# davidfang00/opticalflowdiffusion

Measured on AMD Instinct MI355X. Metric: UNet denoise steps/sec @ 2x436x1024 flow, bs=16, higher is better.
Workload: dtype bf16

## Files before the change

opticalflowdiffusion_amd/csrc/la_fused.hip:

```cpp
#include <cstdlib>
#include "blocks.h"

namespace ofd {

int la_fused_blocks(int n, int B);

typedef __attribute__((ext_vector_type(8))) __bf16 bf16x8;
typedef __attribute__((ext_vector_type(16))) float f32x16;

__device__ __forceinline__ uint32_t la_pack2(float a, float b) { return f2bf2(a, b); }
__device__ __forceinline__ int acc_row(int r, int half) { return (r & 3) + 8 * (r >> 2) + 4 * half; }

__device__ __forceinline__ bf16x8 acc_frag(const f32x16& a, int s2) {
    bf16x8 f;
#pragma unroll
    for (int j = 0; j < 8; ++j) f[j] = (__bf16)a[8 * s2 + j];
    return f;
}

typedef __attribute__((ext_vector_type(4))) unsigned int u32x4;
template <int C>
struct XRaw {
    u32x4 v[C / 16];
};
// ... 327 lines not shown
    __syncthreads();
    const bool use_ws = nparts <= LA_MAX_PARTS;
    float l = 0.0f;
    for (int c0 = grp; c0 < nparts; c0 += 32) {
        float tm[4], tl[4];
#pragma unroll
        for (int k = 0; k < 4; ++k) {
            const size_t o = (size_t)min(c0 + 8 * k, nparts - 1) * 1088;
            tm[k] = base[o + dd];
            tl[k] = base[o + 32 + dd];
        }
#pragma unroll
        for (int k = 0; k < 4; ++k)
            if (c0 + 8 * k < nparts) {
                const float w = __expf(tm[k] - M[dd]);
                if (use_ws) w_s[c0 + 8 * k][dd] = w;
                l += tl[k] * w;
            }
    }
    __syncthreads();
    red[grp][dd] = l;
    __syncthreads();
    if (tid < 32) {
        float t = red[0][tid];
#pragma unroll
        for (int g = 1; g < 8; ++g) t += red[g][tid];
        Linv[tid] = 1.0f / t;
    }
    __syncthreads();
    const int i = blockIdx.y * 256 + tid;
    const int j = i & 7, lane = (i >> 3) & 63, s2 = i >> 9;
    const int d = 16 * s2 + 8 * (j >> 2) + 4 * (lane >> 5) + (j & 3), e = lane & 31;
    float a = 0.0f;
    for (int c0 = 0; c0 < nparts; c0 += 8) {
        float v[8];
#pragma unroll
        for (int k = 0; k < 8; ++k) v[k] = base[(size_t)min(c0 + k, nparts - 1) * 1088 + 64 + d * 32 + e];
        if (use_ws) {
#pragma unroll
            for (int k = 0; k < 8; ++k)
                if (c0 + k < nparts) a += v[k] * w_s[c0 + k][d];
        } else {
            float mc[8];
#pragma unroll
            for (int k = 0; k < 8; ++k) mc[k] = base[(size_t)min(c0 + k, nparts - 1) * 1088 + d];
#pragma unroll
            for (int k = 0; k < 8; ++k)
                if (c0 + k < nparts) a += v[k] * __expf(mc[k] - M[d]);
        }
    }
    ctxfrag[(size_t)bh * 1024 + i] = f2bf(a * Linv[d] * inv_n);
}

template <int C, bool TRAIN>
__global__ void __launch_bounds__(256, C == 64 ? 4 : 2) la_out_fused_kernel(const bf16_t* __restrict__ x, const bf16_t* __restrict__ wq,
                                                           const bf16_t* __restrict__ woutp, const bf16_t* __restrict__ ctxfrag,
                                                           const float* __restrict__ bias, const float* __restrict__ g2,
                                                           bf16_t* __restrict__ y, int n, float eps_pre, float eps_post, float scale,
                                                           const float* __restrict__ g, bf16_t* __restrict__ o2_out) {
    extern __shared__ __attribute__((aligned(16))) unsigned char smem[];
    constexpr int KS = C / 16, RT = C / 32;
    constexpr int WQ_B = (C / 8) * 128 * 16, WO_B = 16 * C * 16, CF_B = 4 * 2 * 64 * 16;
    unsigned char* s_wq = smem;
    unsigned char* s_wo = smem + WQ_B;
    unsigned char* s_cf = s_wo + WO_B;
    float* s_bias = (float*)(s_cf + CF_B);
    float* s_g2 = s_bias + C;
    float* s_g = s_g2 + C;
    const int tid = threadIdx.x, lane = tid & 63, wave = tid >> 6, l31 = lane & 31, half = lane >> 5;
    const int b = blockIdx.y;
    if constexpr (TRAIN)
        for (int i = tid; i < C; i += 256) s_g[i] = g[i];
    for (int i = tid; i < WQ_B / 16; i += 256) ((uint4*)s_wq)[i] = ((const uint4*)wq)[i];
    for (int i = tid; i < WO_B / 16; i += 256) ((uint4*)s_wo)[i] = ((const uint4*)woutp)[i];
    for (int i = tid; i < CF_B / 16; i += 256) ((uint4*)s_cf)[i] = ((const uint4*)(ctxfrag + (size_t)b * 4096))[i];
    for (int i = tid; i < C; i += 256) { s_bias[i] = bias[i]; s_g2[i] = g2[i]; }
    __syncthreads();
    const int wave_id = blockIdx.x * 4 + wave, nw = gridDim.x * 4, ntiles = (n + 31) / 32;

    const bf16_t* xb = x + (size_t)b * n * C;
    XRaw<C> raw_next;
    load_raw_x<C>(xb + (size_t)min(wave_id * 32 + l31, n - 1) * C, raw_next, half);
    for (int tile = wave_id; tile < ntiles; tile += nw) {
        asm volatile("" ::: "memory");
        const int pix = tile * 32 + l31;
        const int pid = min(pix, n - 1);
        const bf16_t* xrow = xb + (size_t)pid * C;
        const XRaw<C> raw = raw_next;
        load_raw_x<C>(xb + (size_t)min((tile + nw) * 32 + l31, n - 1) * C, raw_next, half);
        bf16x8 xs[KS];
        if constexpr (TRAIN) norm_x_gain<C>(raw, eps_pre, s_g, half, xs);
        else norm_x<C>(raw, eps_pre, xs);
        f32x16 acc_o[RT];
#pragma unroll
        for (int rt = 0; rt < RT; ++rt)
#pragma unroll
            for (int r = 0; r < 16; ++r) acc_o[rt][r] = 0.0f;
#pragma unroll
        for (int hd = 0; hd < 4; ++hd) {
            f32x16 qa;
#pragma unroll
            for (int r = 0; r < 16; ++r) qa[r] = 0.0f;
#pragma unroll
            for (int s = 0; s < KS; ++s) {
                const bf16x8 wf = *(const bf16x8*)(s_wq + ((size_t)(2 * s + half) * 128 + hd * 32 + l31) * 16);
                qa = __builtin_amdgcn_mfma_f32_32x32x16_bf16(wf, xs[s], qa, 0, 0, 0);
            }
            if constexpr (TRAIN) {
#pragma unroll
                for (int r = 0; r < 16; ++r) qa[r] = bf2f(f2bf(qa[r]));
            }
            float mx = qa[0];
#pragma unroll
            for (int r = 1; r < 16; ++r) mx = fmaxf(mx, qa[r]);
            mx = fmaxf(mx, __shfl_xor(mx, 32, 64));
            float sum = 0.0f;
#pragma unroll
            for (int r = 0; r < 16; ++r) { qa[r] = __builtin_amdgcn_exp2f(__builtin_fmaf(qa[r], LOG2E, -mx * LOG2E)); sum += qa[r]; }
            sum += __shfl_xor(sum, 32, 64);
            const float k = scale / sum;
#pragma unroll
            for (int r = 0; r < 16; ++r) qa[r] *= k;
            f32x16 oa;
#pragma unroll
            for (int r = 0; r < 16; ++r) oa[r] = 0.0f;
#pragma unroll
            for (int s2 = 0; s2 < 2; ++s2) {
                const bf16x8 cf = *(const bf16x8*)(s_cf + ((size_t)(hd * 2 + s2) * 64 + lane) * 16);
                oa = __builtin_amdgcn_mfma_f32_32x32x16_bf16(cf, acc_frag(qa, s2), oa, 0, 0, 0);
            }
#pragma unroll
            for (int s2 = 0; s2 < 2; ++s2) {
                const bf16x8 of = acc_frag(oa, s2);
#pragma unroll
                for (int rt = 0; rt < RT; ++rt) {
                    const bf16x8 wf = *(const bf16x8*)(s_wo + ((size_t)((hd * 2 + s2) * 2 + half) * C + rt * 32 + l31) * 16);
                    acc_o[rt] = __builtin_amdgcn_mfma_f32_32x32x16_bf16(wf, of, acc_o[rt], 0, 0, 0);
                }
            }
        }
        float sum = 0.0f;
#pragma unroll
        for (int rt = 0; rt < RT; ++rt)
#pragma unroll
            for (int g = 0; g < 4; ++g) {
                const float4 bv = *(const float4*)(s_bias + rt * 32 + 8 * g + 4 * half);
                acc_o[rt][4 * g] += bv.x; acc_o[rt][4 * g + 1] += bv.y; acc_o[rt][4 * g + 2] += bv.z; acc_o[rt][4 * g + 3] += bv.w;
                if constexpr (TRAIN) {
#pragma unroll
                    for (int k = 0; k < 4; ++k) acc_o[rt][4 * g + k] = bf2f(f2bf(acc_o[rt][4 * g + k]));
                }
                sum += (acc_o[rt][4 * g] + acc_o[rt][4 * g + 1]) + (acc_o[rt][4 * g + 2] + acc_o[rt][4 * g + 3]);
            }
        if constexpr (TRAIN) {
            bf16_t* orow = o2_out + ((size_t)b * n + min(pix, n - 1)) * C;
#pragma unroll
            for (int rt = 0; rt < RT; ++rt) store_acc_rows(acc_o[rt], orow + rt * 32, half, pix < n);
        }
        sum += __shfl_xor(sum, 32, 64);
        const float mean = sum * (1.0f / C);
        float q = 0.0f;
#pragma unroll
        for (int rt = 0; rt < RT; ++rt)
#pragma unroll
            for (int r = 0; r < 16; ++r) { acc_o[rt][r] -= mean; q += acc_o[rt][r] * acc_o[rt][r]; }
        q += __shfl_xor(q, 32, 64);
        const float rstd = rsqrtf(q * (1.0f / C) + eps_post);
        {
            const bool ok = pix < n;
            bf16_t* yrow = y + ((size_t)b * n + min(pix, n - 1)) * C;
#pragma unroll
            for (int rt = 0; rt < RT; ++rt)
#pragma unroll
                for (int g = 0; g < 4; g += 2) {
                    const u32x4 xw = raw.v[rt * 2 + (g >> 1)];
                    const uint4 xv = make_uint4(xw[0], xw[1], xw[2], xw[3]);
                    const auto sx = __builtin_amdgcn_permlane32_swap(xv.x, xv.z, false, false);
                    const auto sy = __builtin_amdgcn_permlane32_swap(xv.y, xv.w, false, false);
                    const unsigned xq[2][2] = {{sx[0], sy[0]}, {sx[1], sy[1]}};
                    uint2 qo[2];
#pragma unroll
                    for (int k = 0; k < 2; ++k) {
                        const int c0 = rt * 32 + 8 * (g + k) + 4 * half;
                        const float4 gv = *(const float4*)(s_g2 + c0);
                        const float o0 = acc_o[rt][4 * (g + k)] * rstd * gv.x + bf2f((bf16_t)(xq[k][0] & 0xffffu));
                        const float o1 = acc_o[rt][4 * (g + k) + 1] * rstd * gv.y + bf2f((bf16_t)(xq[k][0] >> 16));
                        const float o2 = acc_o[rt][4 * (g + k) + 2] * rstd * gv.z + bf2f((bf16_t)(xq[k][1] & 0xffffu));
                        const float o3 = acc_o[rt][4 * (g + k) + 3] * rstd * gv.w + bf2f((bf16_t)(xq[k][1] >> 16));
                        qo[k] = make_uint2(la_pack2(o0, o1), la_pack2(o2, o3));
                    }
                    const auto rx = __builtin_amdgcn_permlane32_swap(qo[0].x, qo[1].x, false, false);
                    const auto ry = __builtin_amdgcn_permlane32_swap(qo[0].y, qo[1].y, false, false);
                    if (ok) *(uint4*)(yrow + rt * 32 + 8 * g + 8 * half) = make_uint4(rx[0], ry[0], rx[1], ry[1]);
                }
        }
    }
}

__global__ void __launch_bounds__(256) la_weight_prep_kernel(const float* __restrict__ wqkv, const float* __restrict__ g, const float* __restrict__ wout,
                                                             bf16_t* __restrict__ wq, bf16_t* __restrict__ wkv, bf16_t* __restrict__ woutp, int C) {
    const int total = 512 * C;
    for (int i = blockIdx.x * blockDim.x + threadIdx.x; i < total; i += gridDim.x * blockDim.x) {
        if (i < 128 * C) {
            const int j = i & 7, o = (i >> 3) & 127, c8 = i >> 10, c = c8 * 8 + j;
            wq[i] = f2bf(wqkv[(size_t)o * C + c] * (g ? g[c] : 1.0f));
        } else if (i < 384 * C) {
            const int k = i - 128 * C;
            const int j = k & 7, o = (k >> 3) & 255, c8 = k >> 11, c = c8 * 8 + j;
            wkv[k] = f2bf(wqkv[(size_t)(128 + o) * C + c] * (g ? g[c] : 1.0f));
        } else if (woutp) {
            const int k = i - 384 * C;
            const int j = k & 7, c = (k >> 3) % C, rest = (k >> 3) / C;
            const int hh = rest & 1, s2 = (rest >> 1) & 1, hd = rest >> 2;
            woutp[k] = f2bf(wout[(size_t)c * 128 + hd * 32 + 16 * s2 + 8 * (j >> 2) + 4 * hh + (j & 3)]);
        }
    }
}

constexpr float LA_DEFER = 5.545177f;
constexpr int LA_GX2_CAP = 128;

template <int C>
static int launch_la(const bf16_t* x, const bf16_t* wq, const bf16_t* wkv, const bf16_t* woutp, const float* bias, const float* g2,
                     float* partial, bf16_t* ctxfrag, bf16_t* y, int B, int n, float eps_pre, float eps_post, hipStream_t s) {
    constexpr int LDS1 = (C / 8) * 256 * 16;
    constexpr int LDS2 = (C / 8) * 128 * 16 + 16 * C * 16 + 4 * 2 * 64 * 16 + 2 * C * 4;
    static bool attr = false;
    if (!attr) {
        OFD_HIP(hipFuncSetAttribute((const void*)la_ctx_fused_kernel<C, false>, hipFuncAttributeMaxDynamicSharedMemorySize, LDS1));
        OFD_HIP(hipFuncSetAttribute((const void*)la_out_fused_kernel<C, false>, hipFuncAttributeMaxDynamicSharedMemorySize, LDS2));
        attr = true;
    }
    const int gx = la_fused_blocks(n, B);
    la_ctx_fused_kernel<C, false><<<dim3(gx, B), 256, LDS1, s>>>(x, wkv, partial, n, eps_pre, LA_DEFER, nullptr, nullptr, nullptr);
    la_ctx_combine_frag_kernel<<<dim3(B * 4, 4), 256, 0, s>>>(partial, ctxfrag, gx, 1.0f / (float)n);
    int gx2 = cdiv(cdiv(n, 32), 4 * 4);
    if (gx2 < 1) gx2 = 1;
    const int cap2 = (LA_GX2_CAP * B < 1024) ? 1024 / B : LA_GX2_CAP;
    if (gx2 > cap2) gx2 = cap2;
    la_out_fused_kernel<C, false><<<dim3(gx2, B), 256, LDS2, s>>>(x, wq, woutp, ctxfrag, bias, g2, y, n, eps_pre, eps_post, 0.17677669529663687f, nullptr, nullptr);
    OFD_LAUNCH_CHECK();
    return OFD_OK;
}

void launch_la_ctx_combine(const float* partial, float* ctx, int B, int nparts, float inv_n, float* ml_out, hipStream_t s);

int k_linear_attention_fused_train(const bf16_t* x, const bf16_t* wq, const bf16_t* wkv, const bf16_t* woutp, const float* bias, const float* g_pre,
                                   const float* g2, float* partial, bf16_t* ctxfrag, float* ctx, float* ml, bf16_t* xn, bf16_t* qkv, bf16_t* o2,
                                   bf16_t* y, int B, int n, int C, float eps_pre, float eps_post, hipStream_t s) {
    if (C != 64) { set_error("linear_attention_fused_train: C=%d unsupported", C); return OFD_ERR_ARG; }
    constexpr int LDS1 = (64 / 8) * 256 * 16 + 64 * 4;
    constexpr int LDS2 = (64 / 8) * 128 * 16 + 16 * 64 * 16 + 4 * 2 * 64 * 16 + 3 * 64 * 4;
    static bool attr = false;
    if (!attr) {
        OFD_HIP(hipFuncSetAttribute((const void*)la_ctx_fused_kernel<64, true>, hipFuncAttributeMaxDynamicSharedMemorySize, LDS1));
        OFD_HIP(hipFuncSetAttribute((const void*)la_out_fused_kernel<64, true>, hipFuncAttributeMaxDynamicSharedMemorySize, LDS2));
        attr = true;
    }
    const int gx = la_fused_blocks(n, B);
    la_ctx_fused_kernel<64, true><<<dim3(gx, B), 256, LDS1, s>>>(x, wkv, partial, n, eps_pre, LA_DEFER, g_pre, xn, qkv);
    la_ctx_combine_frag_kernel<<<dim3(B * 4, 4), 256, 0, s>>>(partial, ctxfrag, gx, 1.0f / (float)n);
    launch_la_ctx_combine(partial, ctx, B, gx, 1.0f / (float)n, ml, s);
    int gx2 = cdiv(cdiv(n, 32), 4 * 4);
    if (gx2 < 1) gx2 = 1;
    const int cap2 = (LA_GX2_CAP * B < 1024) ? 1024 / B : LA_GX2_CAP;
    if (gx2 > cap2) gx2 = cap2;
    la_out_fused_kernel<64, true><<<dim3(gx2, B), 256, LDS2, s>>>(x, wq, woutp, ctxfrag, bias, g2, y, n, eps_pre, eps_post, 0.17677669529663687f, g_pre, o2);
    OFD_LAUNCH_CHECK();
    return OFD_OK;
}

int la_fused_blocks(int n, int B) {
    constexpr int total = 256;
    int gx = cdiv(cdiv(n, 32), 8);
    int cap = total / (B < 1 ? 1 : B);
    if (cap < 64) cap = 64;
    if (gx < 1) gx = 1;
    if (gx > cap) gx = cap;
    return gx;
}

int k_la_weight_prep(const float* wqkv, const float* g, const float* wout, bf16_t* wq, bf16_t* wkv, bf16_t* woutp, int C, hipStream_t s) {
    la_weight_prep_kernel<<<cdiv((woutp ? 512 : 384) * C, 256), 256, 0, s>>>(wqkv, g, wout, wq, wkv, woutp, C);
    OFD_LAUNCH_CHECK();
    return OFD_OK;
}

int k_linear_attention_fused(const bf16_t* x, const bf16_t* wq, const bf16_t* wkv, const bf16_t* woutp, const float* bias, const float* g2,
// ... 9 lines not shown
```

opticalflowdiffusion_amd/csrc/unet.hip:

```cpp
#include <cstdlib>
#include "unet_exec.h"

using namespace ofd;

namespace ofd {

float site_eps(const ofd_unet* u, const std::string& site) {
    if (u->cfg.eps_mode == 0) return 1e-5f;
    auto ends = [&](const char* s) { std::string t(s); return site.size() >= t.size() && site.compare(site.size() - t.size(), t.size(), t) == 0; };
    if (ends(".fn.fn.to_out.1")) return 1e-3f;
    if (ends(".0.block1.proj") && site.rfind("downs.", 0) == 0) return 1e-3f;
    if (site == "mid_block1.block1.proj" || site == "final_res_block.block1.proj") return 1e-3f;
    return 1e-5f;
}

static void add_param(ofd_unet* u, const std::string& name, std::vector<int> shape) {
    size_t numel = 1;
    for (int d : shape) numel *= (size_t)d;
    Param p{name, (int)shape.size(), {1, 1, 1, 1}, numel, u->n_param_floats, false};
    for (size_t i = 0; i < shape.size(); ++i) p.shape[i] = shape[i];
    u->pindex[name] = (int)u->params.size();
    u->params.push_back(p);
    u->n_param_floats += (numel + 3) / 4 * 4;
}
// ... 139 lines not shown
    float* a2 = c.train ? c.keepf((size_t)B * Cout) : c.tmpf((size_t)B * Cout);
    float* s2 = c.train ? c.keepf((size_t)B * Cout) : c.tmpf((size_t)B * Cout);
    float* st1 = c.train ? c.keepf((size_t)B * 16) : nullptr;
    float* st2 = c.train ? c.keepf((size_t)B * 16) : nullptr;
    Tensor out = keep_out ? c.keep(Cout, H, W) : c.tmp(Cout, H, W);
    if (c.rc != OFD_OK) return out;
    conv(c, name + ".block1.proj", srcs, h1, nullptr, nullptr, nullptr, nullptr, nullptr, nullptr, p1);
    c.begin(PC_GN, 0, (double)np * 4);
    RUN(k_gn_finalize(p1, B, H, W, Cout, u->P(name + ".block1.norm.weight"), u->P(name + ".block1.norm.bias"), c.ss, u->ss_stride,
                      u->ss_offset.at(name), a1, s1, c.s, st1));
    c.end();
    SrcSpec hs; hs.t = h1;
    constexpr int act1_min = 256;
    constexpr int act1_train_min = 128;
    const int amin = c.train ? act1_train_min : act1_min;
    Tensor act1;
    if (Cout >= amin) {
        act1 = c.tmp(Cout, H, W);
        if (c.rc != OFD_OK) return out;
        c.begin(PC_MISC, 0, (double)B * H * W * Cout * 4.0);
        RUN(k_affine_silu(h1.p, a1, s1, act1.p, B, H, W, Cout, c.s));
        c.end();
        hs.t = act1;
        conv(c, name + ".block2.proj", {hs}, h2, nullptr, nullptr, nullptr, nullptr, nullptr, nullptr, p2);
    } else
    conv(c, name + ".block2.proj", {hs}, h2, a1, s1, nullptr, nullptr, nullptr, nullptr, p2);
    c.begin(PC_GN, 0, (double)np * 4);
    RUN(k_gn_finalize(p2, B, H, W, Cout, u->P(name + ".block2.norm.weight"), u->P(name + ".block2.norm.bias"), nullptr, 0, 0, a2, s2, c.s, st2));
    c.end();
    if (cin != Cout) {
        conv(c, name + ".res_conv", srcs, out, nullptr, nullptr, nullptr, h2.p, a2, s2, nullptr, 0, fc);
    } else {
        c.begin(PC_RESOUT, 0, (double)B * H * W * Cout * 6.0);
        RUN(k_resblock_out(h2.p, a2, s2, in[0].p, out.p, B, H, W, Cout, c.s));
        c.end();
    }
    if (c.train) {
        TapeRec r;
        r.kind = TK_RES; r.name = name; r.srcs = srcs; r.out = out; r.h1 = h1; r.h2 = h2;
        r.a1 = a1; r.s1 = s1; r.a2 = a2; r.s2 = s2; r.st1 = st1; r.st2 = st2; r.act1 = act1;
        u->tape.push_back(r);
    }
    return out;
}

static Tensor linattn(Ctx& c, const std::string& name, Tensor x) {
    ofd_unet* u = c.u;
    const int H = x.H, W = x.W, B = c.B, C = x.C, n = H * W;
    const size_t npix = (size_t)B * n;
    auto fit = u->la_fused.find(name);
    if (fit != u->la_fused.end() && !c.train) {
        const int nparts = la_fused_blocks(n, B);
        float* partial = c.tmpf((size_t)B * 4 * nparts * 1088);
        bf16_t* ctxfrag = (bf16_t*)c.tmpf((size_t)B * 2048);
        Tensor y = c.keep(C, H, W);
        if (c.rc != OFD_OK) return y;
        const bf16_t* base = u->d_labuf + fit->second.first;
        c.begin(PC_LINATTN, npix * 2.0 * (C * 384.0 + 2 * 4 * 32 * 32 + 128.0 * C), (double)npix * C * 2 * 3,
                name + " fused C=" + std::to_string(C) + " @" + std::to_string(H) + "x" + std::to_string(W));
        RUN(k_linear_attention_fused(x.p, base, base + (size_t)128 * C, base + (size_t)384 * C, u->P(name + ".fn.fn.to_out.0.bias"),
                                     u->P(name + ".fn.fn.to_out.1.g"), partial, ctxfrag, y.p, B, n, C, site_eps(u, name + ".fn.norm"),
                                     site_eps(u, name + ".fn.fn.to_out.1"), c.s));
        c.end();
        return y;
    }
    Tensor xn = c.tmp(C, H, W), qkv = c.tmp(384, H, W), ao = c.tmp(128, H, W), o2 = c.tmp(C, H, W);
    const int nparts = la_fwd_parts(B, n);
    if (c.train && fit != u->la_fused.end() && la_train_fused(C)) {
        float* partial = c.tmpf((size_t)B * 4 * nparts * 1088);
        bf16_t* ctxfrag = (bf16_t*)c.tmpf((size_t)B * 2048);
        float* ctx = c.keepf((size_t)B * 4 * 1024);
        float* ml = c.keepf((size_t)B * 4 * 64);
        Tensor y = c.keep(C, H, W);
        if (c.rc != OFD_OK) return y;
        const bf16_t* base = u->d_labuf + fit->second.first;
        c.begin(PC_LINATTN, npix * 2.0 * (C * 640.0 + 2 * 4 * 32 * 32 + 128.0 * C), (double)npix * C * 2 * (2 + 1 + 4 + 2),
                name + " fused (training) C=" + std::to_string(C) + " @" + std::to_string(H) + "x" + std::to_string(W));
        RUN(k_linear_attention_fused_train(x.p, base + (size_t)512 * C, base + (size_t)640 * C, base + (size_t)384 * C, u->P(name + ".fn.fn.to_out.0.bias"),
                                           u->P(name + ".fn.norm.g"), u->P(name + ".fn.fn.to_out.1.g"), partial, ctxfrag, ctx, ml, xn.p, qkv.p, o2.p, y.p,
                                           B, n, C, site_eps(u, name + ".fn.norm"), site_eps(u, name + ".fn.fn.to_out.1"), c.s));
        c.end();
        TapeRec r;
        r.kind = TK_LINATTN; r.name = name; r.x = x; r.xn = xn; r.qkv = qkv; r.ao = ao; r.o2 = o2; r.out = y; r.ctx = ctx; r.ml = ml;
        u->tape.push_back(r);
        return y;
    }
    float* partial = c.tmpf((size_t)B * 4 * nparts * 1088);
    float* ctx = c.train ? c.keepf((size_t)B * 4 * 1024) : c.tmpf((size_t)B * 4 * 1024);
    float* ml = c.train ? c.keepf((size_t)B * 4 * 64) : nullptr;
    Tensor y = c.keep(C, H, W);
    if (c.rc != OFD_OK) return y;
    c.begin(PC_LN, 0, (double)npix * C * 4);
    RUN(k_layernorm_c(x.p, u->P(name + ".fn.norm.g"), nullptr, xn.p, npix, C, site_eps(u, name + ".fn.norm"), c.s));
    c.end();
    SrcSpec s; s.t = xn;
    const bool rq = c.train && la_train_fused(C);
    conv(c, name + ".fn.fn.to_qkv", {s}, qkv, nullptr, nullptr, nullptr, nullptr, nullptr, nullptr, nullptr, rq ? 128 : 0);
    c.begin(PC_LINATTN, 4.0 * npix * 4 * 32 * 32, (double)npix * (384 + 128 + 128) * 2);
    if (C <= 128) {
        const ConvDesc& d = u->convs[u->cindex.at(name + ".fn.fn.to_out.0")];
        bf16_t* ao_out = rq ? nullptr : ao.p;
        const ConvDesc& dq = u->convs[u->cindex.at(name + ".fn.fn.to_qkv")];
        RUN(k_linear_attention_core(qkv.p, partial, ctx, ao_out, B, n, c.s, ml, u->d_wbuf + d.w_off, u->P(name + ".fn.fn.to_out.0.bias"), o2.p, C,
                                    rq ? xn.p : nullptr, rq ? u->d_wbuf + dq.w_off : nullptr));
        c.end();
    } else {
        RUN(k_linear_attention_core(qkv.p, partial, ctx, ao.p, B, n, c.s, ml));
        c.end();
        SrcSpec s2; s2.t = ao;
        conv(c, name + ".fn.fn.to_out.0", {s2}, o2, nullptr, nullptr, nullptr, nullptr, nullptr, nullptr, nullptr);
    }
// ... 159 lines not shown
        }
        u->taps[p + ".3"] = xcur;
    }
    c.reset_scratch();
    const int glue = u->glue_out;
    const bool fuse_fc = !c.train && !u->debug_taps && !glue && u->cfg.out_dim == 2 && dim == 64 && ((long)H * W) % 128 == 0;
    if (fuse_fc) {
        const FcFuse fc{u->P("final_conv.weight"), u->P("final_conv.bias"), out};
        if (c.rc == OFD_OK && !c.dry) {
            if (hipMemsetAsync(out, 0, (size_t)B * 2 * H * W * sizeof(float), c.s) != hipSuccess) { set_error("unet_forward: hipMemsetAsync failed"); c.rc = OFD_ERR_HIP; }
            c.chain_ok = false;
        }
        xcur = resblock(c, "final_res_block", {xcur, r}, dim, true, &fc);
    } else {
        xcur = resblock(c, "final_res_block", {xcur, r}, dim);
        u->taps["final_res_block"] = xcur;
        c.begin(PC_MISC, 2.0 * B * H * W * dim * u->cfg.out_dim, (double)B * H * W * (dim * 2 + u->cfg.out_dim * 4));
        RUN(k_final_conv(xcur.p, u->P("final_conv.weight"), u->P("final_conv.bias"), out, B, H, W, dim, u->cfg.out_dim, c.s, glue, u->glue_div));
        c.end();
    }
    if (c.train) {
        u->ts.B = B; u->ts.H = H; u->ts.W = W; u->ts.t = t; u->ts.ss = c.ss; u->ts.temb = temb; u->ts.temb_silu = temb_silu;
        u->ts.xin = xin; u->ts.r = r; u->ts.xf = xcur; u->ts.persist_used = c.persist_used;
    }
    return c.rc;
}

size_t persist_bytes(const ofd_unet* u, int B, int H, int W) {
    auto T = [&](int C, int h, int w) { return ((size_t)B * h * w * C * 2 + 255) / 256 * 256; };
    const int L = u->L;
    size_t n = T(u->cin_pad, H, W) + T(u->dims[0], H, W);
    int h = H, w = W;
    for (int i = 0; i < L; ++i) {
        n += 3 * T(u->dims[i], h, w);
        if (i < L - 1) { h /= 2; w /= 2; }
        n += T(u->dims[i + 1], h, w);
    }
    n += 3 * T(u->dims[L], h, w);
    for (int i = 0; i < L; ++i) {
        const int co = u->dims[L - i], ci = u->dims[L - 1 - i];
        n += 3 * T(co, h, w);
        if (i < L - 1) { h *= 2; w *= 2; }
        n += T(ci, h, w);
    }
    n += T(u->dims[0], H, W);
    return n + 4096;
}

size_t scratch_bytes(const ofd_unet* u, int B, int H, int W) {
    const size_t px = (size_t)B * H * W;
    const int C = u->dims[0];
    size_t act = px * 2 * (size_t)(3 * C + C + 384 + 128 + C);
    size_t small = 4 * ofd_conv_gn_partial_count(B, H, W, u->dims[u->L]) * 4 + (size_t)B * 4 * ((size_t)(la_fwd_parts(B, H * W) > 256 ? la_fwd_parts(B, H * W) : 256) * 1088 + 1024) * 4 +
                   16 * (size_t)B * u->dims[u->L] * 4 + 64 * 1024;
    return act + small + 64 * 256;
}

size_t small_bytes(const ofd_unet* u, int B) {
    return ((size_t)B * u->ss_stride + 2 * (size_t)B * u->cfg.dim * 4) * 4 + 4096;
}

}

static void drop_graphs(ofd_unet* u);

static void upload_mlp_descs(ofd_unet* u) {
    if (u->cfg.no_time) return;
    std::vector<MlpDesc> descs;
    for (auto& name : u->resblocks) {
        MlpDesc d;
        d.weight = u->P(name + ".mlp.1.weight");
        d.bias = u->P(name + ".mlp.1.bias");
        d.n_out = (int)u->params[u->pindex.at(name + ".mlp.1.bias")].numel;
        d.offset = u->ss_offset.at(name);
        descs.push_back(d);
    }
    if (hipMemcpy(u->d_mlp, descs.data(), descs.size() * sizeof(MlpDesc), hipMemcpyHostToDevice) != hipSuccess)
        set_error("unet: uploading the time-projection descriptors failed");
}

extern "C" int ofd_unet_bind_param_buffer(ofd_unet* u, float* dev_params, size_t floats) {
    OFD_CHECK_ARG(u && dev_params, "unet_bind_param_buffer: null argument");
    OFD_CHECK_ARG(floats >= u->n_param_floats, "unet_bind_param_buffer: %zu floats, need %zu", floats, u->n_param_floats);
    OFD_CHECK_ARG(((uintptr_t)dev_params & 15) == 0, "unet_bind_param_buffer: buffer must be 16-byte aligned");
    if (u->owns_params && u->d_params) (void)hipFree(u->d_params);
    drop_graphs(u);
    if (u->d_prep) { (void)hipFree(u->d_prep); u->d_prep = nullptr; u->n_prep = 0; u->prep_blocks = 0; }
    u->d_params = dev_params;
    u->owns_params = false;
    for (auto& p : u->params) p.set = true;
    upload_mlp_descs(u);
    u->prepared = false;
    u->wt_prepared = false;
    return OFD_OK;
}

extern "C" int ofd_unet_create(const ofd_unet_config* cfg, ofd_unet** out) {
    OFD_CHECK_ARG(cfg && out, "unet_create: null argument");
    OFD_CHECK_ARG(cfg->dim == 64, "unet_create: dim=%d unsupported (the FlowDiffuser UNet is Unet(64), flow_diffuser.py:106)", cfg->dim);
    OFD_CHECK_ARG(cfg->channels >= 1 && cfg->channels <= 48, "unet_create: channels=%d (1..48)", cfg->channels);
    OFD_CHECK_ARG(cfg->out_dim >= 1 && cfg->out_dim <= 16, "unet_create: out_dim=%d (1..16)", cfg->out_dim);
    OFD_CHECK_ARG(cfg->n_levels == 0 || cfg->n_levels == 3 || cfg->n_levels == 4, "unet_create: n_levels=%d (0 or 4: dim_mults (1,2,4,8); 3: (1,2,4))",
                  cfg->n_levels);
    OFD_CHECK_ARG(cfg->n_levels != 3 || cfg->no_time == 1, "unet_create: the three-level UNet (the Autoencoder's) takes no time input (no_time=1)");
    OFD_CHECK_ARG(cfg->eps_mode == 0 || cfg->eps_mode == 1, "unet_create: eps_mode=%d", cfg->eps_mode);
    OFD_CHECK_ARG(cfg->no_time == 0 || cfg->no_time == 1, "unet_create: no_time=%d", cfg->no_time);
// ... 388 lines not shown
```

opticalflowdiffusion_amd/csrc/conv_pc.hip:

```cpp
#include <cstdlib>
#include <type_traits>
#include "conv_common.h"

namespace ofd {

namespace wp {

struct PcCfg {
    using C = Cfg<2, 2>;
    static constexpr int NPROD = C::NTHREADS, XPT = C::XPT;
    static constexpr int WSLOT = FRAGS * 2 * 1024;
    static constexpr int MAX_ITEMS = 512;
    static constexpr int ITEMS_OFF = 2 * C::XB + 2 * WSLOT;
    static constexpr int LDS_BYTES = ITEMS_OFF + MAX_ITEMS * 16;
};

template <bool PRO>
__global__ void __launch_bounds__(512, 2) conv3x3_pc_kernel(const ConvParams P) {
    using C = PcCfg::C;
    constexpr int NPROD = PcCfg::NPROD, XPT = PcCfg::XPT;
    extern __shared__ __attribute__((aligned(16))) unsigned char smem[];
    unsigned char* const wlds = smem + 2 * C::XB;
    const int tid = threadIdx.x;

    const int tiles_y = (P.H + C::ROWS - 1) / C::ROWS;
    const int tpi = P.tiles_x * tiles_y, ntiles = tpi * P.B, ny = P.Cout / C::BN, G = gridDim.x;
    const int nitems = (ntiles + 7) / 8 * 8 * ny;
    const int n32 = P.total_chunks * 2;
    auto decode = [&](int j, int& b, int& oy0, int& ox0, int& cy) -> bool {
        if (j >= nitems) return false;
        const int g = j >> 3;
        cy = ny > 1 ? g % ny : 0;
        int tile = (ny > 1 ? g / ny : g) * 8 + (j & 7);
        if (tile >= ntiles) return false;
        tile = xcd_tile_order(tile, ntiles);
        b = tile / tpi;
        const int t_in = tile - b * tpi;
        oy0 = (t_in / P.tiles_x) * C::ROWS;
        ox0 = (t_in % P.tiles_x) * TW;
        return true;
    };
    const int nit = blockIdx.x < nitems ? min((nitems - 1 - (int)blockIdx.x) / G + 1, PcCfg::MAX_ITEMS) : 0;
    int4* const items = (int4*)(smem + PcCfg::ITEMS_OFF);
    for (int k = tid; k < nit; k += 512) {
        int b_, y_, x_, c_;
        const bool ok = decode(blockIdx.x + k * G, b_, y_, x_, c_);
        items[k] = make_int4(ok ? b_ : -1, y_, x_, c_);
    }
    __syncthreads();
    int nvalid_items = 0;
    if (nit > 0) {
        int lo = 0, hi = nit;
        while (lo < hi) { const int mid = (lo + hi) >> 1; if (items[mid].x >= 0) lo = mid + 1; else hi = mid; }
        nvalid_items = lo;
    }
    const int T = n32 * nvalid_items;
    if (T == 0) return;
    auto item_at = [&](int k, int& b, int& oy0, int& ox0, int& cy) -> bool {
        if (k >= nvalid_items) return false;
        const int4 d = items[k];
        b = __builtin_amdgcn_readfirstlane(d.x); oy0 = __builtin_amdgcn_readfirstlane(d.y);
        ox0 = __builtin_amdgcn_readfirstlane(d.z); cy = __builtin_amdgcn_readfirstlane(d.w);
        return true;
    };

    if (tid >= 256) {
        const int ptid = tid - 256;
        const int c8 = ptid % NC;
        int tyx[XPT];
#pragma unroll
        for (int i = 0; i < XPT; ++i) {
// ... 62 lines not shown
        u4 x0[XPT], x1[XPT], x2[XPT];
        unsigned ok0 = 0, ok1 = 0, ok2 = 0;
        float ps0[8], pb0[8], ps1[8], pb1[8], ps2[8], pb2[8];
        weights_dma(0); stage_advance();
        issue(x0, ok0, ps0, pb0); advance();
        issue(x1, ok1, ps1, pb1); advance();
        issue(x2, ok2, ps2, pb2); advance();
        stage(x0, ok0, ps0, pb0, smem);
        asm volatile("s_waitcnt vmcnt(0)" ::: "memory");
        __syncthreads();
#define PC_STEP(XL, OKL, PSL, PBL, XS, OKS, PSS, PBS, BUF)                                          \
        {                                                                                           \
            if (i >= T) break;                                                                      \
            const bool wd_ = weights_dma(BUF);                  \
            stage_advance();                                                                        \
            issue(XL, OKL, PSL, PBL);                                                               \
            stage(XS, OKS, PSS, PBS, smem + (BUF) * C::XB);                                         \
            advance();                                                                              \
            if (wd_) asm volatile("s_waitcnt vmcnt(%0)" ::"n"(XPT + (PRO ? 4 : 0)) : "memory");     \
            __syncthreads();                                                                        \
            ++i;                                                                                    \
        }
        for (int i = 0; i < T;) {
            PC_STEP(x0, ok0, ps0, pb0, x1, ok1, ps1, pb1, 1)
            PC_STEP(x1, ok1, ps1, pb1, x2, ok2, ps2, pb2, 0)
            PC_STEP(x2, ok2, ps2, pb2, x0, ok0, ps0, pb0, 1)
            PC_STEP(x0, ok0, ps0, pb0, x1, ok1, ps1, pb1, 0)
            PC_STEP(x1, ok1, ps1, pb1, x2, ok2, ps2, pb2, 1)
            PC_STEP(x2, ok2, ps2, pb2, x0, ok0, ps0, pb0, 0)
        }
#undef PC_STEP
        return;
    }

    const int lane = tid & 63, wave = __builtin_amdgcn_readfirstlane(tid >> 6);
    const int l31 = lane & 31, half = lane >> 5;
    const int ns = wave & 1, ph = wave >> 1;
    __builtin_amdgcn_s_setprio(2);

    int ik = 0, b, oy0, ox0, cy;
    item_at(0, b, oy0, ox0, cy);

    f32x16 biasv;
    auto load_bias = [&](int cy_) {
#pragma unroll
        for (int g = 0; g < 4; ++g) {
            const float4 b4 = P.bias ? *(const float4*)(P.bias + cy_ * C::BN + 32 * ns + 8 * g + 4 * half) : make_float4(0.f, 0.f, 0.f, 0.f);
            biasv[4 * g] = b4.x; biasv[4 * g + 1] = b4.y; biasv[4 * g + 2] = b4.z; biasv[4 * g + 3] = b4.w;
        }
    };
    load_bias(cy);
    f32x16 acc[8];

    const int xrow_off = half * C::US + (8 * ph * IW + l31) * 16;
    const unsigned char* const wfrag = wlds + ns * 1024 + lane * 16;
    auto chunk = [&](const int slot, const unsigned char* xbase, auto first_tag) {
        constexpr bool FIRST = decltype(first_tag)::value;
        const unsigned char* xrow = xbase + xrow_off;
#pragma unroll
        for (int g = 0; g < 6; ++g) {
            const int ks = g / 3, kx = g % 3;
            bf16x8 x[10];
#pragma unroll
            for (int jr = 0; jr < 10; ++jr) x[jr] = *(const bf16x8*)(xrow + (jr * IW + kx) * 16 + ks * 2 * C::US);
            bf16x8 a[3];
#pragma unroll
            for (int ky = 0; ky < 3; ++ky) a[ky] = *(const bf16x8*)(wfrag + (slot * FRAGS + g * 3 + ky) * 2048);
#pragma unroll
            for (int r = 0; r < 8; ++r)
#pragma unroll
                for (int ky = 0; ky < 3; ++ky)
                    acc[r] = __builtin_amdgcn_mfma_f32_32x32x16_bf16(a[ky], x[r + ky], (FIRST && g == 0 && ky == 0) ? biasv : acc[r], 0, 0, 0);
        }
    };

    const int tiles8 = (P.H + 7) / 8;
    __syncthreads();
    while (true) {
        int nb, noy0, nox0, ncy;
        const bool nvalid = item_at(ik + 1, nb, noy0, nox0, ncy);
        for (int kc = 0; kc < n32; kc += 2) {
            if (kc == 0) chunk(0, smem, std::true_type{}); else chunk(0, smem, std::false_type{});
            __syncthreads();
            chunk(1, smem + C::XB, std::false_type{});
            __syncthreads();
        }
        __builtin_amdgcn_s_setprio(0);
        float stat[8];
#pragma unroll
        for (int i = 0; i < 8; ++i) stat[i] = 0.0f;
        const int oyb = oy0 + 8 * ph, ox = ox0 + l31, cb = cy * C::BN + 32 * ns;
        const bool okx = ox < P.W;
        const size_t oplane_b = (size_t)P.H * P.W * P.Cout * 2;
        const __amdgpu_buffer_rsrc_t orsrc = __builtin_amdgcn_make_buffer_rsrc((void*)(P.out + (size_t)b * P.H * P.W * P.Cout), 0, (int)oplane_b, 0x00020000);
        const unsigned olane = (unsigned)(((min(oyb, P.H - 1) * P.W + min(ox, P.W - 1)) * P.Cout + cb + 8 * half) * 2);
        const unsigned ostride_b = (unsigned)(P.W * P.Cout * 2);
        const bool full = ox0 + TW <= P.W && oyb + 8 <= P.H && oplane_b < (1ull << 31);
        if (full) {
#pragma unroll
            for (int r = 0; r < 8; ++r) {
                uint2 q[4];
#pragma unroll
                for (int g = 0; g < 4; ++g) {
                    q[g] = make_uint2(f2bf2(acc[r][4 * g], acc[r][4 * g + 1]), f2bf2(acc[r][4 * g + 2], acc[r][4 * g + 3]));
                    if (P.gn_partial) gn_stat_add(q[g], stat[g * 2], stat[g * 2 + 1]);
                }
#pragma unroll
                for (int g = 0; g < 4; g += 2) {
                    const auto rx = __builtin_amdgcn_permlane32_swap(q[g].x, q[g + 1].x, false, false);
                    const auto ry = __builtin_amdgcn_permlane32_swap(q[g].y, q[g + 1].y, false, false);
                    u4 pk = {rx[0], ry[0], rx[1], ry[1]};
                    __builtin_amdgcn_raw_buffer_store_b128(pk, orsrc, (int)olane, (int)(r * ostride_b + 16 * g), 0);
                }
            }
        } else {
        bf16_t* orow = P.out + (((size_t)b * P.H + min(oyb, P.H - 1)) * P.W + min(ox, P.W - 1)) * P.Cout + cb + 8 * half;
        const size_t ostride = (size_t)P.W * P.Cout;
#pragma unroll
        for (int r = 0; r < 8; ++r) {
            const bool ok = okx && oyb + r < P.H;
            uint2 q[4];
#pragma unroll
            for (int g = 0; g < 4; ++g) {
                q[g] = make_uint2(f2bf2(acc[r][4 * g], acc[r][4 * g + 1]), f2bf2(acc[r][4 * g + 2], acc[r][4 * g + 3]));
                if (P.gn_partial && ok) gn_stat_add(q[g], stat[g * 2], stat[g * 2 + 1]);
            }
#pragma unroll
            for (int g = 0; g < 4; g += 2) {
                const auto rx = __builtin_amdgcn_permlane32_swap(q[g].x, q[g + 1].x, false, false);
                const auto ry = __builtin_amdgcn_permlane32_swap(q[g].y, q[g + 1].y, false, false);
                if (ok) *(uint4*)(orow + 8 * g) = make_uint4(rx[0], ry[0], rx[1], ry[1]);
            }
            orow += ostride;
        }
        }
        if (P.gn_partial) gn_partial_store_wave<2, C::BN / 8>(P, stat, b, oy0 / 8 + ph, tiles8, ox0 / TW, ns, cy * C::BN / 8, lane);
        if (!nvalid) break;
        ++ik; b = nb; oy0 = noy0; ox0 = nox0;
        if (ncy != cy) { cy = ncy; load_bias(cy); }
        __builtin_amdgcn_s_setprio(2);
    }
}

static bool pc_serves(const ConvParams& P) {
    for (int i = 0; i < P.n_src; ++i)
        if (P.src[i].mode != 0 && P.src[i].mode != 1) return false;
    return P.Cout % 64 == 0 && plain_epilogue(P) && P.W <= 8160 ;
}

}

int launch_conv3x3_pc(const ConvParams& P, hipStream_t s) {
    using namespace wp;
    using C = PcCfg::C;
    if (!pc_serves(P)) return 1;
    static int cus = 0;
    if (!cus) {
        int dev = 0, n = 0;
        OFD_HIP(hipGetDevice(&dev));
        OFD_HIP(hipDeviceGetAttribute(&n, hipDeviceAttributeMultiprocessorCount, dev));
        OFD_HIP(hipFuncSetAttribute((const void*)conv3x3_pc_kernel<false>, hipFuncAttributeMaxDynamicSharedMemorySize, PcCfg::LDS_BYTES));
        OFD_HIP(hipFuncSetAttribute((const void*)conv3x3_pc_kernel<true>, hipFuncAttributeMaxDynamicSharedMemorySize, PcCfg::LDS_BYTES));
        cus = n / 8 * 8 < 8 ? 8 : n / 8 * 8;
    }
    const int tiles_y = (P.H + C::ROWS - 1) / C::ROWS;
    const int ntiles = P.tiles_x * tiles_y * P.B, ny = P.Cout / C::BN;
    const int nitems = (ntiles + 7) / 8 * 8 * ny;
    const int grid = nitems < cus ? nitems : cus;
    if ((long)grid * PcCfg::MAX_ITEMS < nitems) return 1;
    if (P.in_scale) conv3x3_pc_kernel<true><<<grid, 512, PcCfg::LDS_BYTES, s>>>(P);
    else conv3x3_pc_kernel<false><<<grid, 512, PcCfg::LDS_BYTES, s>>>(P);
    OFD_LAUNCH_CHECK();
    return OFD_OK;
}

}
```

Before: 34.43.

## Fold linear-attention context into output projection weights for inference

Replaces the context-combine kernel with a fold kernel that merges the per-part partials and multiplies the per-head 32x32 context by the output projection, producing a per-sample C x 128 weight fragment. The inference out kernel then applies softmaxed q directly against this folded weight, dropping one MFMA pair per head per tile and the context fragment from LDS. The cost is a larger per-sample folded weight buffer, an extra scalar matmul in the fold kernel, and a new error path when the part count exceeds LA_MAX_PARTS. Rounding also changes slightly because the context and output weights are combined before the bf16 cast.

```diff
diff --git a/opticalflowdiffusion_amd/csrc/la_fused.hip b/opticalflowdiffusion_amd/csrc/la_fused.hip
--- a/opticalflowdiffusion_amd/csrc/la_fused.hip
+++ b/opticalflowdiffusion_amd/csrc/la_fused.hip
@@ -403,6 +403,65 @@
     ctxfrag[(size_t)bh * 1024 + i] = f2bf(a * Linv[d] * inv_n);
 }
 
+template <int C>
+__global__ void __launch_bounds__(1024) la_ctx_fold_kernel(const float* __restrict__ partial, const bf16_t* __restrict__ woutp,
+                                                           bf16_t* __restrict__ mfrag, int nparts, float inv_n) {
+    __shared__ float red[32][32], M[32], Linv[32], w_s[LA_MAX_PARTS][32], ctx_s[32][33], wo_s[C][33];
+    const int tid = threadIdx.x, bh = blockIdx.x, hd = bh & 3, dd = tid & 31, grp = tid >> 5;
+    const float* base = partial + (size_t)bh * nparts * 1088;
+    for (int i = tid; i < C * 32; i += 1024) {
+        const int c = i >> 5, e = i & 31;
+        wo_s[c][e] = bf2f(woutp[((size_t)((hd * 2 + (e >> 4)) * 2 + ((e >> 2) & 1)) * C + c) * 8 + ((e >> 3) & 1) * 4 + (e & 3)]);
+    }
+    float mx = -3.0e38f;
+    for (int c0 = grp; c0 < nparts; c0 += 32) mx = fmaxf(mx, base[(size_t)c0 * 1088 + dd]);
+    red[grp][dd] = mx;
+    __syncthreads();
+    if (tid < 32) {
+        float m = red[0][tid];
+#pragma unroll
+        for (int g = 1; g < 32; ++g) m = fmaxf(m, red[g][tid]);
+        M[tid] = m;
+    }
+    __syncthreads();
+    float l = 0.0f;
+    for (int c0 = grp; c0 < nparts; c0 += 32) {
+        const float w = __expf(base[(size_t)c0 * 1088 + dd] - M[dd]);
+        w_s[c0][dd] = w;
+        l += base[(size_t)c0 * 1088 + 32 + dd] * w;
+    }
+    __syncthreads();
+    red[grp][dd] = l;
+    __syncthreads();
+    if (tid < 32) {
+        float t = red[0][tid];
+#pragma unroll
+        for (int g = 1; g < 32; ++g) t += red[g][tid];
+        Linv[tid] = inv_n / t;
+    }
+    __syncthreads();
+    float a = 0.0f;
+    for (int c0 = 0; c0 < nparts; c0 += 8) {
+        float v[8];
+#pragma unroll
+        for (int k = 0; k < 8; ++k) v[k] = base[(size_t)min(c0 + k, nparts - 1) * 1088 + 64 + tid];
+#pragma unroll
+        for (int k = 0; k < 8; ++k)
+            if (c0 + k < nparts) a += v[k] * w_s[c0 + k][grp];
+    }
+    ctx_s[grp][dd] = a * Linv[grp];
+    __syncthreads();
+    bf16_t* out = mfrag + (size_t)bh * 32 * C;
+    for (int i = tid; i < 32 * C; i += 1024) {
+        const int j = i & 7, c = (i >> 3) % C, rest = (i >> 3) / C;
+        const int d = 16 * (rest >> 1) + 8 * (j >> 2) + 4 * (rest & 1) + (j & 3);
+        float t = 0.0f;
+#pragma unroll
+        for (int e = 0; e < 32; ++e) t += wo_s[c][e] * ctx_s[d][e];
+        out[i] = f2bf(t);
+    }
+}
+
 template <int C, bool TRAIN>
 __global__ void __launch_bounds__(256, C == 64 ? 4 : 2) la_out_fused_kernel(const bf16_t* __restrict__ x, const bf16_t* __restrict__ wq,
                                                            const bf16_t* __restrict__ woutp, const bf16_t* __restrict__ ctxfrag,
@@ -411,7 +470,7 @@
                                                            const float* __restrict__ g, bf16_t* __restrict__ o2_out) {
     extern __shared__ __attribute__((aligned(16))) unsigned char smem[];
     constexpr int KS = C / 16, RT = C / 32;
-    constexpr int WQ_B = (C / 8) * 128 * 16, WO_B = 16 * C * 16, CF_B = 4 * 2 * 64 * 16;
+    constexpr int WQ_B = (C / 8) * 128 * 16, WO_B = 16 * C * 16, CF_B = TRAIN ? 4 * 2 * 64 * 16 : 0;
     unsigned char* s_wq = smem;
     unsigned char* s_wo = smem + WQ_B;
     unsigned char* s_cf = s_wo + WO_B;
@@ -423,8 +482,12 @@
     if constexpr (TRAIN)
         for (int i = tid; i < C; i += 256) s_g[i] = g[i];
     for (int i = tid; i < WQ_B / 16; i += 256) ((uint4*)s_wq)[i] = ((const uint4*)wq)[i];
-    for (int i = tid; i < WO_B / 16; i += 256) ((uint4*)s_wo)[i] = ((const uint4*)woutp)[i];
-    for (int i = tid; i < CF_B / 16; i += 256) ((uint4*)s_cf)[i] = ((const uint4*)(ctxfrag + (size_t)b * 4096))[i];
+    if constexpr (TRAIN) {
+        for (int i = tid; i < WO_B / 16; i += 256) ((uint4*)s_wo)[i] = ((const uint4*)woutp)[i];
+        for (int i = tid; i < CF_B / 16; i += 256) ((uint4*)s_cf)[i] = ((const uint4*)(ctxfrag + (size_t)b * 4096))[i];
+    } else {
+        for (int i = tid; i < WO_B / 16; i += 256) ((uint4*)s_wo)[i] = ((const uint4*)(ctxfrag + (size_t)b * 128 * C))[i];
+    }
     for (int i = tid; i < C; i += 256) { s_bias[i] = bias[i]; s_g2[i] = g2[i]; }
     __syncthreads();
     const int wave_id = blockIdx.x * 4 + wave, nw = gridDim.x * 4, ntiles = (n + 31) / 32;
@@ -473,16 +536,18 @@
 #pragma unroll
             for (int r = 0; r < 16; ++r) qa[r] *= k;
             f32x16 oa;
-#pragma unroll
-            for (int r = 0; r < 16; ++r) oa[r] = 0.0f;
+            if constexpr (TRAIN) {
+#pragma unroll
+                for (int r = 0; r < 16; ++r) oa[r] = 0.0f;
+#pragma unroll
+                for (int s2 = 0; s2 < 2; ++s2) {
+                    const bf16x8 cf = *(const bf16x8*)(s_cf + ((size_t)(hd * 2 + s2) * 64 + lane) * 16);
+                    oa = __builtin_amdgcn_mfma_f32_32x32x16_bf16(cf, acc_frag(qa, s2), oa, 0, 0, 0);
+                }
+            }
 #pragma unroll
             for (int s2 = 0; s2 < 2; ++s2) {
-                const bf16x8 cf = *(const bf16x8*)(s_cf + ((size_t)(hd * 2 + s2) * 64 + lane) * 16);
-                oa = __builtin_amdgcn_mfma_f32_32x32x16_bf16(cf, acc_frag(qa, s2), oa, 0, 0, 0);
-            }
-#pragma unroll
-            for (int s2 = 0; s2 < 2; ++s2) {
-                const bf16x8 of = acc_frag(oa, s2);
+                const bf16x8 of = TRAIN ? acc_frag(oa, s2) : acc_frag(qa, s2);
 #pragma unroll
                 for (int rt = 0; rt < RT; ++rt) {
                     const bf16x8 wf = *(const bf16x8*)(s_wo + ((size_t)((hd * 2 + s2) * 2 + half) * C + rt * 32 + l31) * 16);
@@ -575,7 +640,7 @@
 static int launch_la(const bf16_t* x, const bf16_t* wq, const bf16_t* wkv, const bf16_t* woutp, const float* bias, const float* g2,
                      float* partial, bf16_t* ctxfrag, bf16_t* y, int B, int n, float eps_pre, float eps_post, hipStream_t s) {
     constexpr int LDS1 = (C / 8) * 256 * 16;
-    constexpr int LDS2 = (C / 8) * 128 * 16 + 16 * C * 16 + 4 * 2 * 64 * 16 + 2 * C * 4;
+    constexpr int LDS2 = (C / 8) * 128 * 16 + 16 * C * 16 + 2 * C * 4;
     static bool attr = false;
     if (!attr) {
         OFD_HIP(hipFuncSetAttribute((const void*)la_ctx_fused_kernel<C, false>, hipFuncAttributeMaxDynamicSharedMemorySize, LDS1));
@@ -584,7 +649,8 @@
     }
     const int gx = la_fused_blocks(n, B);
     la_ctx_fused_kernel<C, false><<<dim3(gx, B), 256, LDS1, s>>>(x, wkv, partial, n, eps_pre, LA_DEFER, nullptr, nullptr, nullptr);
-    la_ctx_combine_frag_kernel<<<dim3(B * 4, 4), 256, 0, s>>>(partial, ctxfrag, gx, 1.0f / (float)n);
+    if (gx > LA_MAX_PARTS) { set_error("linear_attention_fused: %d parts per sample", gx); return OFD_ERR_ARG; }
+    la_ctx_fold_kernel<C><<<B * 4, 1024, 0, s>>>(partial, woutp, ctxfrag, gx, 1.0f / (float)n);
     int gx2 = cdiv(cdiv(n, 32), 4 * 4);
     if (gx2 < 1) gx2 = 1;
     const int cap2 = (LA_GX2_CAP * B < 1024) ? 1024 / B : LA_GX2_CAP;
diff --git a/opticalflowdiffusion_amd/csrc/unet.hip b/opticalflowdiffusion_amd/csrc/unet.hip
--- a/opticalflowdiffusion_amd/csrc/unet.hip
+++ b/opticalflowdiffusion_amd/csrc/unet.hip
@@ -215,11 +215,11 @@
     if (fit != u->la_fused.end() && !c.train) {
         const int nparts = la_fused_blocks(n, B);
         float* partial = c.tmpf((size_t)B * 4 * nparts * 1088);
-        bf16_t* ctxfrag = (bf16_t*)c.tmpf((size_t)B * 2048);
+        bf16_t* ctxfrag = (bf16_t*)c.tmpf((size_t)B * 64 * C);
         Tensor y = c.keep(C, H, W);
         if (c.rc != OFD_OK) return y;
         const bf16_t* base = u->d_labuf + fit->second.first;
-        c.begin(PC_LINATTN, npix * 2.0 * (C * 384.0 + 2 * 4 * 32 * 32 + 128.0 * C), (double)npix * C * 2 * 3,
+        c.begin(PC_LINATTN, npix * 2.0 * (C * 384.0 + 4 * 32 * 32 + 128.0 * C), (double)npix * C * 2 * 3,
                 name + " fused C=" + std::to_string(C) + " @" + std::to_string(H) + "x" + std::to_string(W));
         RUN(k_linear_attention_fused(x.p, base, base + (size_t)128 * C, base + (size_t)384 * C, u->P(name + ".fn.fn.to_out.0.bias"),
                                      u->P(name + ".fn.fn.to_out.1.g"), partial, ctxfrag, y.p, B, n, C, site_eps(u, name + ".fn.norm"),
@@ -485,6 +485,7 @@
     const int C = u->dims[0];
     size_t act = px * 2 * (size_t)(3 * C + C + 384 + 128 + C);
     size_t small = 4 * ofd_conv_gn_partial_count(B, H, W, u->dims[u->L]) * 4 + (size_t)B * 4 * ((size_t)(la_fwd_parts(B, H * W) > 256 ? la_fwd_parts(B, H * W) : 256) * 1088 + 1024) * 4 +
+                   (size_t)B * 128 * 128 * 2 +
                    16 * (size_t)B * u->dims[u->L] * 4 + 64 * 1024;
     return act + small + 64 * 256;
 }
```

New measurement: 34.58 (median of 5 runs). Within noise of the previous version (+0.4%).

## Interleave epilogue row stores with last-chunk MFMAs in persistent conv3x3 kernel

Applied to the files above, without the earlier changes.

During the final K-chunk of each work item, the conv kernel now converts, stores and accumulates GroupNorm stats for output rows 0-5 right after their accumulators finish their last MFMA. Only the remaining rows are handled after the loop. This hides epilogue conversion and global-store latency behind the tail MFMAs rather than running the epilogue serially after the main loop. The drain path is on by default via an env knob, and it adds register pressure and per-row address recomputation in the partial-tile path.

```diff
diff --git a/opticalflowdiffusion_amd/csrc/conv_pc.hip b/opticalflowdiffusion_amd/csrc/conv_pc.hip
--- a/opticalflowdiffusion_amd/csrc/conv_pc.hip
+++ b/opticalflowdiffusion_amd/csrc/conv_pc.hip
@@ -16,7 +16,7 @@
 };
 
 template <bool PRO>
-__global__ void __launch_bounds__(512, 2) conv3x3_pc_kernel(const ConvParams P) {
+__global__ void __launch_bounds__(512, 2) conv3x3_pc_kernel(const ConvParams P, const int drain) {
     using C = PcCfg::C;
     constexpr int NPROD = PcCfg::NPROD, XPT = PcCfg::XPT;
     extern __shared__ __attribute__((aligned(16))) unsigned char smem[];
@@ -185,10 +185,73 @@
     load_bias(cy);
     f32x16 acc[8];
 
+    constexpr int TAIL = 6;
+    const int tiles8 = (P.H + 7) / 8;
+    struct Epi {
+        __amdgpu_buffer_rsrc_t rsrc;
+        unsigned olane;
+        bool full;
+        int k;
+    };
+    auto epi_setup = [&](const int k) -> Epi {
+        int b_, oy0_, ox0_, cy_;
+        item_at(k, b_, oy0_, ox0_, cy_);
+        Epi E;
+        const int oyb = oy0_ + 8 * ph, ox = ox0_ + l31, cb = cy_ * C::BN + 32 * ns;
+        const size_t oplane_b = (size_t)P.H * P.W * P.Cout * 2;
+        E.rsrc = __builtin_amdgcn_make_buffer_rsrc((void*)(P.out + (size_t)b_ * P.H * P.W * P.Cout), 0, (int)oplane_b, 0x00020000);
+        E.olane = (unsigned)(((min(oyb, P.H - 1) * P.W + min(ox, P.W - 1)) * P.Cout + cb + 8 * half) * 2);
+        E.full = ox0_ + TW <= P.W && oyb + 8 <= P.H && oplane_b < (1ull << 31);
+        E.k = k;
+        return E;
+    };
+    auto cvt_row = [&](const f32x16& v, uint2 (&q)[4]) {
+#pragma unroll
+        for (int g = 0; g < 4; ++g) q[g] = make_uint2(f2bf2(v[4 * g], v[4 * g + 1]), f2bf2(v[4 * g + 2], v[4 * g + 3]));
+    };
+    auto finish_row = [&](const Epi& E, const int r, const uint2 (&q)[4], float (&stat)[8]) {
+        if (E.full) {
+#pragma unroll
+            for (int g = 0; g < 4; ++g)
+                if (P.gn_partial) gn_stat_add(q[g], stat[g * 2], stat[g * 2 + 1]);
+#pragma unroll
+            for (int g = 0; g < 4; g += 2) {
+                const auto rx = __builtin_amdgcn_permlane32_swap(q[g].x, q[g + 1].x, false, false);
+                const auto ry = __builtin_amdgcn_permlane32_swap(q[g].y, q[g + 1].y, false, false);
+                u4 pk = {rx[0], ry[0], rx[1], ry[1]};
+                __builtin_amdgcn_raw_buffer_store_b128(pk, E.rsrc, (int)E.olane, (int)(r * (unsigned)(P.W * P.Cout * 2) + 16 * g), 0);
+            }
+        } else {
+            int b_, oy0_, ox0_, cy_;
+            item_at(E.k, b_, oy0_, ox0_, cy_);
+            const int oyb = oy0_ + 8 * ph, ox = ox0_ + l31;
+            const bool ok = ox < P.W && oyb + r < P.H;
+            bf16_t* const orow = P.out + (((size_t)b_ * P.H + min(oyb, P.H - 1)) * P.W + min(ox, P.W - 1)) * P.Cout + cy_ * C::BN + 32 * ns + 8 * half;
+#pragma unroll
+            for (int g = 0; g < 4; ++g)
+                if (P.gn_partial && ok) gn_stat_add(q[g], stat[g * 2], stat[g * 2 + 1]);
+#pragma unroll
+            for (int g = 0; g < 4; g += 2) {
+                const auto rx = __builtin_amdgcn_permlane32_swap(q[g].x, q[g + 1].x, false, false);
+                const auto ry = __builtin_amdgcn_permlane32_swap(q[g].y, q[g + 1].y, false, false);
+                if (ok) *(uint4*)(orow + (size_t)r * P.W * P.Cout + 8 * g) = make_uint4(rx[0], ry[0], rx[1], ry[1]);
+            }
+        }
+    };
+    auto partial_store = [&](const Epi& E, float (&stat)[8]) {
+        if (!P.gn_partial) return;
+        int b_, oy0_, ox0_, cy_;
+        item_at(E.k, b_, oy0_, ox0_, cy_);
+        gn_partial_store_wave<2, C::BN / 8>(P, stat, b_, oy0_ / 8 + ph, tiles8, ox0_ / TW, ns, cy_ * C::BN / 8, lane);
+    };
+    Epi E;
+    float stat[8];
+
     const int xrow_off = half * C::US + (8 * ph * IW + l31) * 16;
     const unsigned char* const wfrag = wlds + ns * 1024 + lane * 16;
-    auto chunk = [&](const int slot, const unsigned char* xbase, auto first_tag) {
-        constexpr bool FIRST = decltype(first_tag)::value;
+    auto chunk = [&](const int slot, const unsigned char* xbase, auto kind_tag, const bool drains) {
+        constexpr int KIND = decltype(kind_tag)::value;
+        constexpr bool FIRST = KIND == 1;
         const unsigned char* xrow = xbase + xrow_off;
 #pragma unroll
         for (int g = 0; g < 6; ++g) {
@@ -200,78 +263,54 @@
 #pragma unroll
             for (int ky = 0; ky < 3; ++ky) a[ky] = *(const bf16x8*)(wfrag + (slot * FRAGS + g * 3 + ky) * 2048);
 #pragma unroll
-            for (int r = 0; r < 8; ++r)
+            for (int r = 0; r < 8; ++r) {
 #pragma unroll
                 for (int ky = 0; ky < 3; ++ky)
                     acc[r] = __builtin_amdgcn_mfma_f32_32x32x16_bf16(a[ky], x[r + ky], (FIRST && g == 0 && ky == 0) ? biasv : acc[r], 0, 0, 0);
-        }
-    };
-
-    const int tiles8 = (P.H + 7) / 8;
+                if (KIND == 2 && g == 5 && r >= 1 && r <= TAIL && drains) {
+                    if (r == 1) {
+                        E = epi_setup(ik);
+#pragma unroll
+                        for (int i = 0; i < 8; ++i) stat[i] = 0.0f;
+                    }
+                    uint2 q[4];
+                    cvt_row(acc[r - 1], q);
+                    finish_row(E, r - 1, q, stat);
+                }
+            }
+        }
+    };
+    using Kind0 = std::integral_constant<int, 0>; using Kind1 = std::integral_constant<int, 1>; using Kind2 = std::integral_constant<int, 2>;
+
     __syncthreads();
     while (true) {
         int nb, noy0, nox0, ncy;
         const bool nvalid = item_at(ik + 1, nb, noy0, nox0, ncy);
         for (int kc = 0; kc < n32; kc += 2) {
-            if (kc == 0) chunk(0, smem, std::true_type{}); else chunk(0, smem, std::false_type{});
+            if (kc == 0) chunk(0, smem, Kind1{}, false); else chunk(0, smem, Kind0{}, false);
             __syncthreads();
-            chunk(1, smem + C::XB, std::false_type{});
+            const bool last = drain && kc + 2 == n32;
+            chunk(1, smem + C::XB, Kind2{}, last);
             __syncthreads();
         }
         __builtin_amdgcn_s_setprio(0);
-        float stat[8];
-#pragma unroll
-        for (int i = 0; i < 8; ++i) stat[i] = 0.0f;
-        const int oyb = oy0 + 8 * ph, ox = ox0 + l31, cb = cy * C::BN + 32 * ns;
-        const bool okx = ox < P.W;
-        const size_t oplane_b = (size_t)P.H * P.W * P.Cout * 2;
-        const __amdgpu_buffer_rsrc_t orsrc = __builtin_amdgcn_make_buffer_rsrc((void*)(P.out + (size_t)b * P.H * P.W * P.Cout), 0, (int)oplane_b, 0x00020000);
-        const unsigned olane = (unsigned)(((min(oyb, P.H - 1) * P.W + min(ox, P.W - 1)) * P.Cout + cb + 8 * half) * 2);
-        const unsigned ostride_b = (unsigned)(P.W * P.Cout * 2);
-        const bool full = ox0 + TW <= P.W && oyb + 8 <= P.H && oplane_b < (1ull << 31);
-        if (full) {
-#pragma unroll
-            for (int r = 0; r < 8; ++r) {
-                uint2 q[4];
-#pragma unroll
-                for (int g = 0; g < 4; ++g) {
-                    q[g] = make_uint2(f2bf2(acc[r][4 * g], acc[r][4 * g + 1]), f2bf2(acc[r][4 * g + 2], acc[r][4 * g + 3]));
-                    if (P.gn_partial) gn_stat_add(q[g], stat[g * 2], stat[g * 2 + 1]);
-                }
-#pragma unroll
-                for (int g = 0; g < 4; g += 2) {
-                    const auto rx = __builtin_amdgcn_permlane32_swap(q[g].x, q[g + 1].x, false, false);
-                    const auto ry = __builtin_amdgcn_permlane32_swap(q[g].y, q[g + 1].y, false, false);
-                    u4 pk = {rx[0], ry[0], rx[1], ry[1]};
-                    __builtin_amdgcn_raw_buffer_store_b128(pk, orsrc, (int)olane, (int)(r * ostride_b + 16 * g), 0);
-                }
-            }
-        } else {
-        bf16_t* orow = P.out + (((size_t)b * P.H + min(oyb, P.H - 1)) * P.W + min(ox, P.W - 1)) * P.Cout + cb + 8 * half;
-        const size_t ostride = (size_t)P.W * P.Cout;
+        if (!drain) {
+            E = epi_setup(ik);
+#pragma unroll
+            for (int i = 0; i < 8; ++i) stat[i] = 0.0f;
+        }
 #pragma unroll
         for (int r = 0; r < 8; ++r) {
-            const bool ok = okx && oyb + r < P.H;
+            if (r < TAIL && drain) continue;
             uint2 q[4];
-#pragma unroll
-            for (int g = 0; g < 4; ++g) {
-                q[g] = make_uint2(f2bf2(acc[r][4 * g], acc[r][4 * g + 1]), f2bf2(acc[r][4 * g + 2], acc[r][4 * g + 3]));
-                if (P.gn_partial && ok) gn_stat_add(q[g], stat[g * 2], stat[g * 2 + 1]);
-            }
-#pragma unroll
-            for (int g = 0; g < 4; g += 2) {
-                const auto rx = __builtin_amdgcn_permlane32_swap(q[g].x, q[g + 1].x, false, false);
-                const auto ry = __builtin_amdgcn_permlane32_swap(q[g].y, q[g + 1].y, false, false);
-                if (ok) *(uint4*)(orow + 8 * g) = make_uint4(rx[0], ry[0], rx[1], ry[1]);
-            }
-            orow += ostride;
-        }
-        }
-        if (P.gn_partial) gn_partial_store_wave<2, C::BN / 8>(P, stat, b, oy0 / 8 + ph, tiles8, ox0 / TW, ns, cy * C::BN / 8, lane);
+            cvt_row(acc[r], q);
+            finish_row(E, r, q, stat);
+        }
+        partial_store(E, stat);
         if (!nvalid) break;
+        __builtin_amdgcn_s_setprio(2);
         ++ik; b = nb; oy0 = noy0; ox0 = nox0;
         if (ncy != cy) { cy = ncy; load_bias(cy); }
-        __builtin_amdgcn_s_setprio(2);
     }
 }
 
@@ -301,8 +340,9 @@
     const int nitems = (ntiles + 7) / 8 * 8 * ny;
     const int grid = nitems < cus ? nitems : cus;
     if ((long)grid * PcCfg::MAX_ITEMS < nitems) return 1;
-    if (P.in_scale) conv3x3_pc_kernel<true><<<grid, 512, PcCfg::LDS_BYTES, s>>>(P);
-    else conv3x3_pc_kernel<false><<<grid, 512, PcCfg::LDS_BYTES, s>>>(P);
+    const int drain = env_int("OFD_CONV_PC_DRAIN", 1);
+    if (P.in_scale) conv3x3_pc_kernel<true><<<grid, 512, PcCfg::LDS_BYTES, s>>>(P, drain);
+    else conv3x3_pc_kernel<false><<<grid, 512, PcCfg::LDS_BYTES, s>>>(P, drain);
     OFD_LAUNCH_CHECK();
     return OFD_OK;
 }
```

Measured after the change: 33.29 before, 33.47 after (median of 6 runs). No clear change (+0.5%).
